# Sunscreen-tech/Sunscreen

Hardware: NVIDIA H100
Metric: ciphertext mul+relin/sec (higher is better)
Workload: dtype u64

## Files before the change

### sunscreen_b200/csrc/b200_bfv.cu

```cuda
#include "../../include/b200_bfv.h"
#include "bfv_body.cuh"
#include "host_ctx.h"
#include "ntt_body.cuh"
#include "ntt_fp_body.cuh"
#include <atomic>
#include <cstdio>
#include <cstdlib>
#include <cstring>
#ifdef B200_EMU_HEADER
#include B200_EMU_HEADER
#else
#include <cuda_runtime.h>
#include <map>
#include <string>
#include <vector>
struct B200TraceRec
{
    const char *name;
    cudaEvent_t e0, e1;
};
static int g_trace_on = -1;
static std::vector<B200TraceRec> g_trace;
static const char *g_trace_name = nullptr;
static inline bool trace_on()
// ... 128 lines not shown
    const int r = (int)(t % R);
    const long long item = t / R;
    const PrimeDev P = ld_prime(r < L.k ? &L.q[r] : &L.bsk[r - L.k]);
    const int Pn = square ? sa : sa + sb;
    const int Dn = square ? 3 : sa + sb - 1;
    const u64 *A = ext + ((item * Pn) * R + r) * n;
    u64 *Dp = D + ((item * Dn) * R + r) * n;
    if (!square && (sa > 4 || sb > 4))
    {
        tensor_coeff_general(P, A, R * n, sa, A + (long long)sa * R * n, R * n, sb, Dp, R * n, c);
        return;
    }
    if (L.fp)
    {
        const double *pd = r < L.k ? &L.dq[2 * r] : &L.dbsk[2 * (r - L.k)];
        const double p = __ldg(pd), pinv = __ldg(pd + 1);
        if (square)
            square_coeff_fp(p, pinv, A, R * n, Dp, R * n, c);
        else
            tensor_coeff_fp(p, pinv, A, R * n, sa, A + (long long)sa * R * n, R * n, sb, Dp, R * n, c);
        return;
    }
    if (square)
        square_coeff(P, A, R * n, Dp, R * n, c);
    else
        tensor_coeff(P, A, R * n, sa, A + (long long)sa * R * n, R * n, sb, Dp, R * n, c);
}

template <int K>
__global__ void scale_kernel(const ScaleIntC<K> L, const u64 *D, int Dn, u64 *dst0, int split, u64 *dst1, long long n,
                             long long total)
{
    const long long idx = GLOBAL_IDX();
    if (idx >= total)
        return;
    const int R = K + L.nBsk;
    const long long c = idx % n;
    const long long t = idx / n;
    const int m = (int)(t % Dn);
    const long long item = t / Dn;
    const u64 *src = D + ((item * Dn + m) * R) * n;
    u64 *dst = m < split ? dst0 + ((item * split + m) * K) * n : dst1 + ((item * (Dn - split) + (m - split)) * K) * n;
    scale_coeff<K>(L, src, dst, n, c);
}

template <int K>
__global__ void ksmac_kernel(const PrimeDev *primes, const NttPrimeFp *fprimes, int use_fp, int special_idx, int key_rows,
                             const u64 *ks1, const u64 *key, u64 *ks2, long long n, long long total)
{
    const long long idx = GLOBAL_IDX();
    if (idx >= total)
        return;
    const long long c = idx % n;
    const long long t = idx / n;
    const int I = (int)(t % (K + 1));
    const long long item = t / (K + 1);
    const int prime_idx = I < K ? I : special_idx;
    const int key_res = I < K ? I : key_rows - 1;
    const PrimeDev P = ld_prime(&primes[prime_idx]);
    const u64 *ops = ks1 + ((item * (K + 1) + I) * K) * n;
    const u64 *kp = key + (long long)key_res * n;
    u64 *o0 = ks2 + ((item * 2 + 0) * (K + 1) + I) * n;
    u64 *o1 = ks2 + ((item * 2 + 1) * (K + 1) + I) * n;
    if (use_fp)
    {
        const double p = __ldg(&fprimes[prime_idx].p), pinv = __ldg(&fprimes[prime_idx].pinv);
        ksmac_coeff_fp<K>(p, pinv, ops, n, kp, 2LL * key_rows * n, (long long)key_rows * n, o0, o1, c);
        return;
    }
    ksmac_coeff<K>(P, ops, n, kp, 2LL * key_rows * n, (long long)key_rows * n, o0, o1, c);
}

#ifdef B200_EMU_HEADER
struct b200_u64x2
{
    u64 x, y;
};
static inline b200_u64x2 ldg2(const u64 *p) { return b200_u64x2{ p[0], p[1] }; }
static inline void stg2(u64 *p, u64 a, u64 b)
{
    p[0] = a;
    p[1] = b;
}
#else
typedef ulonglong2 b200_u64x2;
__device__ __forceinline__ ulonglong2 ldg2(const u64 *p) { return __ldg(reinterpret_cast<const b200_u64x2 *>(p)); }
__device__ __forceinline__ void stg2(u64 *p, u64 a, u64 b) { *reinterpret_cast<ulonglong2 *>(p) = make_ulonglong2(a, b); }
#endif

template <int K>
__global__ void lift_kernel_v2(const LiftFpC<K> L, const u64 *a, int sa, const u64 *b, int sb, u64 *ext, long long n, long long total)
{
    const long long idx = GLOBAL_IDX();
    if (idx >= total)
        return;
    const int P = sa + sb;
    const long long hn = n >> 1;
    const long long c = (idx % hn) * 2;
    const long long t = idx / hn;
    const int p = (int)(t % P);
    const long long item = t / P;
    const int R = K + L.nBsk;
    const u64 *src = p < sa ? a + (item * sa + p) * K * n : b + (item * sb + (p - sa)) * K * n;
    u64 *dst = ext + ((item * P + p) * R + K) * n;
    u64 xs[2][K], zs[2][K + 2];
#pragma unroll
    for (int i = 0; i < K; i++)
    {
        const b200_u64x2 v = ldg2(src + i * n + c);
        xs[0][i] = v.x;
        xs[1][i] = v.y;
    }
    lift_coeff_fp<K>(L, xs[0], zs[0], 1, 0);
    lift_coeff_fp<K>(L, xs[1], zs[1], 1, 0);
#pragma unroll
    for (int j = 0; j < K + 2; j++)
        if (j < L.nBsk)
            stg2(dst + j * n + c, zs[0][j], zs[1][j]);
}

__global__ void tensor_kernel_v2(const LevelDev L, const u64 *ext, u64 *D, long long n, long long total, int square)
{
    const long long idx = GLOBAL_IDX();
    if (idx >= total)
        return;
    const int R = L.k + L.nBsk;
    const long long hn = n >> 1;
    const long long c = (idx % hn) * 2;
    const long long t = idx / hn;
    const int r = (int)(t % R);
    const long long item = t / R;
    const double *pd = r < L.k ? &L.dq[2 * r] : &L.dbsk[2 * (r - L.k)];
    const double p = __ldg(pd), pinv = __ldg(pd + 1);
    const int Pn = square ? 2 : 4;
    const u64 *A = ext + ((item * Pn) * R + r) * n + c;
    u64 *Dp = D + ((item * 3) * R + r) * n + c;
    const long long ps = (long long)R * n;
    const b200_u64x2 a0 = ldg2(A), a1 = ldg2(A + ps);
    u64 in[2][4], out[2][3];
    in[0][0] = a0.x; in[1][0] = a0.y; in[0][1] = a1.x; in[1][1] = a1.y;
    if (!square)
    {
        const b200_u64x2 b0 = ldg2(A + 2 * ps), b1 = ldg2(A + 3 * ps);
        in[0][2] = b0.x; in[1][2] = b0.y; in[0][3] = b1.x; in[1][3] = b1.y;
    }
#pragma unroll
    for (int u = 0; u < 2; u++)
    {
        if (square)
            square_coeff_fp(p, pinv, in[u], 1, out[u], 1, 0);
        else
            tensor_coeff_fp(p, pinv, in[u], 1, 2, in[u] + 2, 1, 2, out[u], 1, 0);
    }
#pragma unroll
    for (int m = 0; m < 3; m++)
        stg2(Dp + m * ps, out[0][m], out[1][m]);
}

template <int K>
__global__ void scale_kernel_v2(const ScaleFpC<K> L, const u64 *D, int Dn, u64 *dst0, int split, u64 *dst1, long long n, long long total)
{
    const long long idx = GLOBAL_IDX();
    if (idx >= total)
        return;
    const int R = K + L.nBsk;
    const long long hn = n >> 1;
    const long long c = (idx % hn) * 2;
    const long long t = idx / hn;
    const int m = (int)(t % Dn);
    const long long item = t / Dn;
    const u64 *src = D + ((item * Dn + m) * R) * n + c;
    u64 *dst = (m < split ? dst0 + ((item * split + m) * K) * n : dst1 + ((item * (Dn - split) + (m - split)) * K) * n) + c;
    u64 in[2][2 * K + 2], out[2][K];
#pragma unroll
    for (int i = 0; i < 2 * K + 2; i++)
        if (i < R)
        {
            const b200_u64x2 v = ldg2(src + i * n);
            in[0][i] = v.x;
            in[1][i] = v.y;
        }
    scale_coeff_fp<K>(L, in[0], out[0], 1, 0);
    scale_coeff_fp<K>(L, in[1], out[1], 1, 0);
#pragma unroll
    for (int i = 0; i < K; i++)
        stg2(dst + i * n, out[0][i], out[1][i]);
}

template <int K>
__global__ void ksmac_kernel_v2(const NttPrimeFp *fprimes, int special_idx, int key_rows, const u64 *ks1, const u64 *key, u64 *ks2,
                                long long n, long long total)
{
    const long long idx = GLOBAL_IDX();
    if (idx >= total)
        return;
    const long long hn = n >> 1;
    const long long c = (idx % hn) * 2;
    const long long t = idx / hn;
    const int I = (int)(t % (K + 1));
    const long long item = t / (K + 1);
    const int prime_idx = I < K ? I : special_idx;
    const int key_res = I < K ? I : key_rows - 1;
    const double p = __ldg(&fprimes[prime_idx].p), pinv = __ldg(&fprimes[prime_idx].pinv);
    const u64 *ops = ks1 + ((item * (K + 1) + I) * K) * n + c;
    const u64 *kp = key + (long long)key_res * n + c;
    double acc[2][2] = { { 0.0, 0.0 }, { 0.0, 0.0 } };
#pragma unroll
    for (int J = 0; J < K; J++)
    {
        const b200_u64x2 x = ldg2(ops + J * n);
        const b200_u64x2 k0 = ldg2(kp + J * 2LL * key_rows * n), k1 = ldg2(kp + J * 2LL * key_rows * n + (long long)key_rows * n);
        const double x0 = fp_from_u64(x.x), x1 = fp_from_u64(x.y);
        acc[0][0] = B200_DADD(acc[0][0], fp_mulmod2(x0, fp_from_u64(k0.x), p, pinv));
        acc[0][1] = B200_DADD(acc[0][1], fp_mulmod2(x0, fp_from_u64(k1.x), p, pinv));
        acc[1][0] = B200_DADD(acc[1][0], fp_mulmod2(x1, fp_from_u64(k0.y), p, pinv));
        acc[1][1] = B200_DADD(acc[1][1], fp_mulmod2(x1, fp_from_u64(k1.y), p, pinv));
    }
    u64 *o0 = ks2 + ((item * 2 + 0) * (K + 1) + I) * n + c;
    u64 *o1 = ks2 + ((item * 2 + 1) * (K + 1) + I) * n + c;
    stg2(o0, fp_to_canonical(acc[0][0], p, pinv), fp_to_canonical(acc[1][0], p, pinv));
    stg2(o1, fp_to_canonical(acc[0][1], p, pinv), fp_to_canonical(acc[1][1], p, pinv));
}

template <int K>
__global__ void ksmoddown_kernel(const PrimeDev *primes, int special_idx, const u64 *inv_qsp, const u64 *ks2,
                                 const u64 *base0, long long base0_stride, const u64 *base1, long long base1_stride,
                                 u64 *dst, long long dst_item_stride, long long n, long long total)
{
    const long long idx = GLOBAL_IDX();
    if (idx >= total)
        return;
    const long long c = idx % n;
    const long long t = idx / n;
    const int comp = (int)(t & 1);
    const long long item = t >> 1;
    const PrimeDev SP = ld_prime(&primes[special_idx]);
    const u64 *acc = ks2 + ((item * 2 + comp) * (K + 1)) * n;
    const u64 *base = comp == 0 ? (base0 ? base0 + item * base0_stride : nullptr)
                                : (base1 ? base1 + item * base1_stride : nullptr);
    u64 *d = dst + item * dst_item_stride + (long long)comp * K * n;
    ksmoddown_coeff<K>(primes, SP, inv_qsp, acc, n, base, d, c);
}

template <int K>
__global__ void ksmoddown_kernel_v2(const PrimeDev *primes, int special_idx, const u64 *inv_qsp, const u64 *ks2,
                                    const u64 *base0, long long base0_stride, const u64 *base1, long long base1_stride,
                                    u64 *dst, long long dst_item_stride, long long n, long long total)
{
    const long long idx = GLOBAL_IDX();
    if (idx >= total)
        return;
    const long long hn = n >> 1;
    const long long c = (idx % hn) * 2;
    const long long t = idx / hn;
    const int comp = (int)(t & 1);
    const long long item = t >> 1;
    const PrimeDev SP = ld_prime(&primes[special_idx]);
    const u64 *acc = ks2 + ((item * 2 + comp) * (K + 1)) * n + c;
    const u64 *base = comp == 0 ? (base0 ? base0 + item * base0_stride : nullptr) : (base1 ? base1 + item * base1_stride : nullptr);
    u64 *d = dst + item * dst_item_stride + (long long)comp * K * n + c;
    const u64 half = SP.p >> 1;
    const b200_u64x2 sp = ldg2(acc + (long long)K * n);
    u64 s0 = sp.x + half, s1 = sp.y + half;
    s0 = s0 >= SP.p ? s0 - SP.p : s0;
    s1 = s1 >= SP.p ? s1 - SP.p : s1;
#pragma unroll
    for (int i = 0; i < K; i++)
    {
        const PrimeDev Q = ld_prime(&primes[i]);
        const u64 h = barrett64(half, Q.p, Q.r1);
        const u64 w = B200_LDG(&inv_qsp[2 * i]), wq = B200_LDG(&inv_qsp[2 * i + 1]);
        const b200_u64x2 a = ldg2(acc + (long long)i * n);
        u64 v0 = a.x + (Q.p - barrett64(s0, Q.p, Q.r1)) + h;
        u64 v1 = a.y + (Q.p - barrett64(s1, Q.p, Q.r1)) + h;
        v0 = shoup_mul(v0, w, wq, Q.p);
        v1 = shoup_mul(v1, w, wq, Q.p);
        if (base)
        {
            const b200_u64x2 b = ldg2(base + c + (long long)i * n);
            v0 = add_mod(v0, b.x, Q.p);
            v1 = add_mod(v1, b.y, Q.p);
        }
        stg2(d + (long long)i * n, v0, v1);
    }
}

template <int K>
__global__ void modswitch_kernel(const PrimeDev *primes, const u64 *inv_qlast, const u64 *src, u64 *dst, long long n,
                                 long long total)
{
    const long long idx = GLOBAL_IDX();
    if (idx >= total)
        return;
    const long long c = idx % n;
    const long long poly = idx / n;
    modswitch_coeff<K>(primes, inv_qlast, src + poly * K * n, n, dst + poly * (K - 1) * n, c);
}

__global__ void galois_kernel(const PrimeDev *primes, int k, const u64 *in2, u64 *out2, u64 *tmp, int logn, u32 g,
                              long long total)
{
    const long long idx = GLOBAL_IDX();
    if (idx >= total)
        return;
    const long long n = 1LL << logn;
    const long long c = idx & (n - 1);
    const long long t = idx >> logn;
    const int r = (int)(t % k);
    const long long u = t / k;
    const int poly = (int)(u & 1);
    const long long item = u >> 1;
    const u64 p = __ldg(&primes[r].p);
    const u64 *src = in2 + ((item * 2 + poly) * k + r) * n;
    u64 *dst = poly == 0 ? out2 + ((item * 2) * k + r) * n : tmp + (item * k + r) * n;
    galois_coeff(p, src, dst, logn, g, c);
}

__global__ void addsub_kernel(const PrimeDev *primes, int k, const u64 *a, const u64 *b, u64 *out, int logn, int mode,
                              long long total)
{
    const long long idx = GLOBAL_IDX();
    if (idx >= total)
        return;
    const int r = (int)((idx >> logn) % k);
    const u64 p = __ldg(&primes[r].p);
    const u64 x = a[idx];
    u64 v;
    if (mode == 0)
        v = add_mod(x, b[idx], p);
    else if (mode == 1)
        v = sub_mod(x, b[idx], p);
    else
        v = neg_mod(x, p);
    out[idx] = v;
}

__global__ void expand_signed_kernel(const PrimeDev *primes, int k, const long long *vals, u64 *out, int logn, long long total)
{
    const long long idx = GLOBAL_IDX();
    if (idx >= total)
        return;
    const long long c = idx & ((1LL << logn) - 1);
    const long long row = idx >> logn;
    const int r = (int)(row % k);
    const long long poly = row / k;
    const long long v = vals[(poly << logn) + c];
    out[idx] = v < 0 ? __ldg(&primes[r].p) + (u64)v : (u64)v;
}

__global__ void dyadic_plain_kernel(const PrimeDev *primes, int k, int size, const u64 *x, const u64 *y, long long pb,
                                    u64 *out, int logn, long long total)
{
    const long long idx = GLOBAL_IDX();
    if (idx >= total)
        return;
    const long long n = 1LL << logn;
    const long long c = idx & (n - 1);
    const long long t = idx >> logn;
    const int r = (int)(t % k);
    const long long u = t / k;
    const long long item = u / size;
    const PrimeDev P = ld_prime(&primes[r]);
    const u64 yv = y[((item % pb) * k + r) * n + c];
    u64 lo, hi;
    mul128(x[idx], yv, lo, hi);
    out[idx] = barrett128(lo, hi, P.p, P.r0, P.r1);
}
// ... 919 lines not shown
    for (int b = 0; b < Lh.nB; b++)
    {
        C.sk_c[2 * b] = Lh.sk_c[b].w;
        C.sk_c[2 * b + 1] = Lh.sk_c[b].wq;
        C.sk_mat_msk[b] = Lh.sk_mat_msk[b];
    }
    C.sk_inv_b_msk = Lh.sk_inv_b_msk;
    return C;
}
template <int K>
static LiftFpC<K> make_lift_fpc(const b200_ctx *ctx, int level)
{
    const LevelFpHost &H = ctx->fp_levels[level];
    LiftFpC<K> C;
    memset(&C, 0, sizeof(C));
    C.nBsk = H.nBsk;
    C.neg_inv_q_mod_mt = H.neg_inv_q_mod_mt;
    for (int i = 0; i < K; i++)
        C.mt[i] = H.lift_mt[i];
    std::copy(H.dq.begin(), H.dq.end(), C.dq);
    std::copy(H.dbsk.begin(), H.dbsk.end(), C.dbsk);
    std::copy(H.lift_c.begin(), H.lift_c.end(), C.c);
    std::copy(H.lift_mat.begin(), H.lift_mat.end(), C.mat);
    std::copy(H.lift_qm.begin(), H.lift_qm.end(), C.qm);
    return C;
}
template <int K>
static ScaleFpC<K> make_scale_fpc(const b200_ctx *ctx, int level)
{
    const LevelFpHost &H = ctx->fp_levels[level];
    ScaleFpC<K> C;
    memset(&C, 0, sizeof(C));
    C.nB = H.nB;
    C.nBsk = H.nBsk;
    std::copy(H.dq.begin(), H.dq.end(), C.dq);
    std::copy(H.dbsk.begin(), H.dbsk.end(), C.dbsk);
    std::copy(H.scale_c.begin(), H.scale_c.end(), C.c);
    std::copy(H.scale_tq.begin(), H.scale_tq.end(), C.tq);
    std::copy(H.scale_mat.begin(), H.scale_mat.end(), C.mat);
    std::copy(H.sk_c.begin(), H.sk_c.end(), C.sk_c);
    for (int i = 0; i < K; i++)
        for (int b = 0; b < H.nB; b++)
        {
            C.sk_mat_q[2 * (i * (K + 1) + b)] = H.sk_mat_q[2 * (i * H.nB + b)];
            C.sk_mat_q[2 * (i * (K + 1) + b) + 1] = H.sk_mat_q[2 * (i * H.nB + b) + 1];
        }
    std::copy(H.sk_mat_msk.begin(), H.sk_mat_msk.end(), C.sk_mat_msk);
    std::copy(H.prod_b_q.begin(), H.prod_b_q.end(), C.prod_b_q);
    std::copy(H.negprod_b_q.begin(), H.negprod_b_q.end(), C.negprod_b_q);
    C.inv_b_msk[0] = H.inv_b_msk[0];
    C.inv_b_msk[1] = H.inv_b_msk[1];
    return C;
}

static const int EB = 256;

static int check_level(b200_ctx *ctx, int level)
{
    if (!ctx)
        return fail(B200_E_NULL, "null context");
    if (level < 0 || level >= (int)ctx->levels.size())
        return fail(B200_E_INVALID, "level out of range");
    return 0;
}

static int dense_job(b200_ctx *ctx, const std::string &key, const std::vector<int> &prime, JobDesc *jd)
{
    std::vector<long long> off(prime.size());
    for (size_t i = 0; i < prime.size(); i++)
        off[i] = (long long)i * (long long)ctx->n;
    return get_job(ctx, key, prime, off, off, jd);
}

static std::vector<int> row_primes(b200_ctx *ctx, int level, bool with_bsk)
{
    const LevelHost &Lh = ctx->host->levels[level];
    std::vector<int> r(Lh.q_idx);
    if (with_bsk)
        r.insert(r.end(), Lh.bsk_idx.begin(), Lh.bsk_idx.end());
    return r;
}

static int multiply_core(b200_ctx *ctx, int level, const u64 *a, int sa, const u64 *b, int sb, bool square, u64 *dst0,
                         int split, u64 *dst1, long long batch, cudaStream_t s)
{
    const LevelDev &L = ctx->levels[level];
    const LevelHost &Lh = ctx->host->levels[level];
    const long long n = (long long)ctx->n;
    const int k = L.k, R = k + L.nBsk;
    const int P = square ? sa : sa + sb;
    const int Dn = square ? 3 : sa + sb - 1;
    Scratch scr(ctx, s);
    u64 *ext = nullptr, *D = nullptr;
    int rc;
    if ((rc = scr.get((size_t)batch * P * R * n, &ext)))
        return rc;
    if ((rc = scr.get((size_t)batch * Dn * R * n, &D)))
        return rc;
    bool clustered = false;
    {
        if (L.fp)
        {
            const long long total = batch * P * (n >> 1);
            DISPATCH_K(k, B200_LAUNCH(lift_kernel_v2<KK>, blocks_for(total, EB), EB, 0, s, make_lift_fpc<KK>(ctx, level), a, sa,
                                      square ? a : b, square ? 0 : sb, ext, n, total));
        }
        else
        {
            const long long total = batch * P * n;
            DISPATCH_K(k, B200_LAUNCH(lift_kernel<KK>, blocks_for(total, EB), EB, 0, s, make_lift_intc<KK>(ctx, level), a, sa,
                                      square ? a : b, square ? 0 : sb, ext, n, total));
        }
        ctx->launches++;
    }
#ifndef B200_EMU_HEADER
    static const bool want_cluster = !(std::getenv("B200_MUL_CLUSTER") && std::getenv("B200_MUL_CLUSTER")[0] == '0') &&
                                     !std::getenv("B200_TENSOR_FUSION");
    if (want_cluster && !square && sa == 2 && sb == 2 && L.fp && ctx->mul_clusters > 0 && ctx->logn <= 13 &&
        4LL * R * batch > 2LL * ctx->sm_count)
    {
        JobDesc jd;
        if ((rc = get_job(ctx, "mulcl:" + std::to_string(level), row_primes(ctx, level, true), {}, {}, &jd)))
            return rc;
        if (static_fp_ok(ctx, jd))
        {
            if (4LL * R * batch > 0x7fffffffLL)
                return fail(B200_E_INVALID, "batch too large for one multiply launch");
            NttJob job;
            memset(&job, 0, sizeof(job));
            job.logn = ctx->logn;
            job.slots = R;
            job.slot_prime = jd.d_prime;
            job.primes = ctx->d_ntt_primes;
            job.fprimes = ctx->d_fp_primes;
            job.items = batch;
            cudaEvent_t t0 = nullptr, t1 = nullptr;
            if (trace_on())
            {
                cudaEventCreate(&t0);
                cudaEventCreate(&t1);
                cudaEventRecord(t0, s);
            }
            const int crc = b200_mul_cluster(ctx->logn, job, a, b, ext, D, k, s);
            if (crc)
                return fail(B200_E_CUDA, std::string("mul_cluster_kernel: ") + cudaGetErrorString((cudaError_t)crc));
            if (t0)
            {
                cudaEventRecord(t1, s);
                g_trace.push_back(B200TraceRec{ "mul_cluster_kernel", t0, t1 });
            }
            ctx->launches++;
            clustered = true;
        }
    }
#endif
    if (!clustered)
    {
        std::vector<int> prime;
        std::vector<long long> so, dof;
        NttAlt alt;
        for (int which = 0; which < (square ? 1 : 2); which++)
        {
            const int sz = which == 0 ? sa : sb;
            const int p0 = which == 0 ? 0 : sa;
            for (int p = 0; p < sz; p++)
                for (int r = 0; r < k; r++)
                {
                    prime.push_back(Lh.q_idx[r]);
                    so.push_back(((long long)p * k + r) * n);
                    dof.push_back(((long long)(p0 + p) * R + r) * n);
                }
            alt.end[which] = (int)prime.size();
            alt.src[which] = which == 0 ? a : b;
            alt.stride[which] = (long long)sz * k * n;
        }
        if (square)
            alt.end[1] = alt.end[0];
        for (int p = 0; p < P; p++)
            for (int j = 0; j < L.nBsk; j++)
            {
                prime.push_back(Lh.bsk_idx[j]);
                so.push_back(((long long)p * R + k + j) * n);
                dof.push_back(((long long)p * R + k + j) * n);
            }
        JobDesc jd;
        std::string key = "mulfwd:" + std::to_string(level) + ":" + std::to_string(sa) + ":" + std::to_string(square ? 0 : sb);
        if ((rc = get_job(ctx, key, prime, so, dof, &jd)))
            return rc;
        if ((rc = launch_ntt<true>(ctx, jd, ext, (long long)P * R * n, ext, (long long)P * R * n, batch, 0, s, nullptr, &alt)))
            return rc;
    }
    if (!clustered)
    {
        std::vector<int> rows = row_primes(ctx, level, true), prime;
        for (int m = 0; m < Dn; m++)
            prime.insert(prime.end(), rows.begin(), rows.end());
        JobDesc jd;
        if ((rc = dense_job(ctx, "muld:" + std::to_string(level) + ":" + std::to_string(Dn), prime, &jd)))
            return rc;
        static const bool want_fuse = std::getenv("B200_TENSOR_FUSION") != nullptr;
        const bool fuse = want_fuse && L.fp && static_fp_ok(ctx, jd);
        TensorArgs ta;
        if (fuse)
        {
            ta.mode = square ? 2 : 1;
            ta.sa = sa;
            ta.sb = sb;
            ta.rows = R;
            ta.src = ext;
        }
        else
        {
            if (L.fp && (square || (sa == 2 && sb == 2)))
            {
                const long long total = batch * R * (n >> 1);
                B200_LAUNCH(tensor_kernel_v2, blocks_for(total, EB), EB, 0, s, L, ext, D, n, total, square ? 1 : 0);
            }
            else
            {
                const long long total = batch * R * n;
                B200_LAUNCH(tensor_kernel, blocks_for(total, EB), EB, 0, s, L, ext, sa, sb, D, n, total, square ? 1 : 0);
            }
            ctx->launches++;
        }
        if ((rc = launch_ntt<false>(ctx, jd, D, (long long)Dn * R * n, D, (long long)Dn * R * n, batch, 0, s, fuse ? &ta : nullptr)))
            return rc;
    }
    {
        if (L.fp)
        {
            const long long total = batch * Dn * (n >> 1);
            DISPATCH_K(k, B200_LAUNCH(scale_kernel_v2<KK>, blocks_for(total, EB), EB, 0, s, make_scale_fpc<KK>(ctx, level), D, Dn,
                                      dst0, split, dst1, n, total));
        }
        else
        {
            const long long total = batch * Dn * n;
            DISPATCH_K(k, B200_LAUNCH(scale_kernel<KK>, blocks_for(total, EB), EB, 0, s, make_scale_intc<KK>(ctx, level), D, Dn, dst0,
                                      split, dst1, n, total));
        }
        ctx->launches++;
    }
    CU_TRY(cudaGetLastError());
    return 0;
}

static int keyswitch_core(b200_ctx *ctx, int level, const u64 *d, long long d_stride, const u64 *key, const u64 *base0,
                          long long base0_stride, const u64 *base1, long long base1_stride, u64 *dst,
                          long long dst_stride, long long batch, cudaStream_t s)
{
    if (!ctx->host->using_keyswitching || level < 1)
        return fail(B200_E_LOGIC, "keyswitching is not supported by the context");
    const LevelDev &L = ctx->levels[level];
    const LevelHost &Lh = ctx->host->levels[level];
    const long long n = (long long)ctx->n;
    const int k = L.k;
    const int Kkey = ctx->host->K;
    const int special = Kkey - 1;
    Scratch scr(ctx, s);
    u64 *ks1 = nullptr, *ks2 = nullptr;
    int rc;
    if ((rc = scr.get((size_t)batch * 2 * (k + 1) * n, &ks2)))
        return rc;
    bool clustered = false;
#ifndef B200_EMU_HEADER
    static const bool want_cluster = !(std::getenv("B200_KS_CLUSTER") && std::getenv("B200_KS_CLUSTER")[0] == '0');
    if (want_cluster && L.fp && ctx->logn <= 13 && k >= 2 && k <= 8 && ctx->ks_clusters[k] > 0 &&
        (long long)k * (k + 1) * batch > 2LL * ctx->sm_count)
    {
        std::vector<int> prime;
        for (int I = 0; I <= k; I++)
            prime.push_back(I < k ? Lh.q_idx[I] : special);
        JobDesc jd;
        if ((rc = get_job(ctx, "kscl:" + std::to_string(level), prime, {}, {}, &jd)))
            return rc;
        if (static_fp_ok(ctx, jd))
        {
            if ((long long)k * (k + 1) * batch > 0x7fffffffLL)
                return fail(B200_E_INVALID, "batch too large for one key-switch launch");
            NttJob job;
            memset(&job, 0, sizeof(job));
            job.logn = ctx->logn;
            job.slots = k + 1;
            job.slot_prime = jd.d_prime;
            job.primes = ctx->d_ntt_primes;
            job.fprimes = ctx->d_fp_primes;
            job.reduce_input = 1;
            job.items = batch;
            cudaEvent_t t0 = nullptr, t1 = nullptr;
            if (trace_on())
            {
                cudaEventCreate(&t0);
                cudaEventCreate(&t1);
                cudaEventRecord(t0, s);
            }
            const int crc = b200_ks_cluster(ctx->logn, job, d, d_stride, key, Kkey, ks2, k, s);
            if (crc)
                return fail(B200_E_CUDA, std::string("ks_cluster_kernel: ") + cudaGetErrorString((cudaError_t)crc));
            if (t0)
            {
                cudaEventRecord(t1, s);
                g_trace.push_back(B200TraceRec{ "ks_cluster_kernel", t0, t1 });
            }
            ctx->launches++;
            clustered = true;
        }
    }
#endif
    if (!clustered && (rc = scr.get((size_t)batch * (k + 1) * k * n, &ks1)))
        return rc;
    if (!clustered)
    {
        std::vector<int> prime;
        std::vector<long long> so, dof;
        for (int I = 0; I <= k; I++)
            for (int J = 0; J < k; J++)
            {
                prime.push_back(I < k ? Lh.q_idx[I] : special);
                so.push_back((long long)J * n);
                dof.push_back(((long long)I * k + J) * n);
            }
        JobDesc jd;
        if ((rc = get_job(ctx, "ks1:" + std::to_string(level), prime, so, dof, &jd)))
            return rc;
        if ((rc = launch_ntt<true>(ctx, jd, d, d_stride, ks1, (long long)(k + 1) * k * n, batch, 1, s)))
            return rc;
    }
    if (!clustered)
    {
        bool done = false;
#ifndef B200_EMU_HEADER
        static const bool want_tma = !(std::getenv("B200_KSMAC_TMA") && std::getenv("B200_KSMAC_TMA")[0] == '0');
        if (want_tma && b200_ksmac_tma_supported(n, k))
        {
            if (trace_on())
                g_trace_name = "ksmac_tma_kernel";
            cudaEvent_t t0 = nullptr, t1 = nullptr;
            if (trace_on())
            {
                cudaEventCreate(&t0);
                cudaEventCreate(&t1);
                cudaEventRecord(t0, s);
            }
            const int rc2 = b200_ksmac_tma(k, L.fp ? 1 : 0, ctx->d_primes, ctx->d_fp_primes, special, Kkey, ks1, key, ks2, n, batch,
                                           ctx->sm_count, s);
            if (rc2 > 0)
                return fail(B200_E_CUDA, std::string("ksmac_tma_kernel: ") + cudaGetErrorString((cudaError_t)rc2));
            if (rc2 == 0)
            {
                done = true;
                if (t0)
                {
                    cudaEventRecord(t1, s);
                    g_trace.push_back(B200TraceRec{ "ksmac_tma_kernel", t0, t1 });
                    g_trace_name = nullptr;
                }
            }
        }
#endif
        if (done)
            ;
        else if (L.fp)
        {
            const long long total = batch * (k + 1) * (n >> 1);
            DISPATCH_K(k, B200_LAUNCH(ksmac_kernel_v2<KK>, blocks_for(total, EB), EB, 0, s, ctx->d_fp_primes, special, Kkey, ks1, key,
                                      ks2, n, total));
        }
        else
        {
            const long long total = batch * (k + 1) * n;
            DISPATCH_K(k, B200_LAUNCH(ksmac_kernel<KK>, blocks_for(total, EB), EB, 0, s, ctx->d_primes, ctx->d_fp_primes,
                                      (int)(L.fp != 0), special, Kkey, ks1, key, ks2, n, total));
        }
        ctx->launches++;
    }
    if (!clustered)
    {
        std::vector<int> prime;
        for (int comp = 0; comp < 2; comp++)
            for (int I = 0; I <= k; I++)
                prime.push_back(I < k ? Lh.q_idx[I] : special);
        JobDesc jd;
        if ((rc = dense_job(ctx, "ks2:" + std::to_string(level), prime, &jd)))
            return rc;
        if ((rc = launch_ntt<false>(ctx, jd, ks2, 2LL * (k + 1) * n, ks2, 2LL * (k + 1) * n, batch, 0, s)))
            return rc;
    }
    {
        const long long total = batch * 2 * (n >> 1);
        DISPATCH_K(k, B200_LAUNCH(ksmoddown_kernel_v2<KK>, blocks_for(total, EB), EB, 0, s, ctx->d_primes, special, ctx->d_inv_qsp, ks2,
                                                                                base0, base0_stride, base1, base1_stride,
                                                                                dst, dst_stride, n, total));
        ctx->launches++;
    }
    CU_TRY(cudaGetLastError());
    return 0;
}

extern "C" {

const char *b200_last_error(void) { return g_err.c_str(); }

int b200_device_count(void)
{
    int c = 0;
    if (cudaGetDeviceCount(&c) != cudaSuccess)
        return 0;
    return c;
}

int b200_ctx_create(uint64_t n, const uint64_t *coeff_modulus, uint64_t count, uint64_t plain_modulus, int device,
                    b200_ctx **out)
{
    if (!coeff_modulus || !out)
        return fail(B200_E_NULL, "null argument");
    *out = nullptr;
    std::unique_ptr<b200_ctx> ctx(new b200_ctx());
    try
    {
        std::vector<b200::u64> mods(coeff_modulus, coeff_modulus + count);
        ctx->host.reset(new BfvHostContext((size_t)n, mods, plain_modulus));
    }
    catch (const std::invalid_argument &e)
    {
        return fail(B200_E_INVALID, e.what());
    }
    catch (const std::logic_error &e)
    {
        return fail(B200_E_LOGIC, e.what());
    }
    catch (const std::exception &e)
    {
        return fail(B200_E_INVALID, e.what());
    }
    ctx->n = ctx->host->n;
    ctx->logn = ctx->host->logn;
    int ndev = 0;
    cudaError_t e = cudaGetDeviceCount(&ndev);
    if (e != cudaSuccess || ndev == 0)
        return fail(B200_E_CUDA, "no CUDA device available: the CUDA backend has no CPU fallback");
    if (device < 0 || device >= ndev)
        return fail(B200_E_INVALID, "device index out of range");
    CU_TRY(cudaSetDevice(device));
    ctx->device = device;
    cudaDeviceProp prop;
    CU_TRY(cudaGetDeviceProperties(&prop, device));
    ctx->sm_count = prop.multiProcessorCount;
    ctx->ntt_split = ctx->logn >= 15 ? (std::getenv("B200_NTT_SPLIT") ? atoi(std::getenv("B200_NTT_SPLIT")) : 2) : 0;
    if (ctx->ntt_split < 1 && ctx->logn >= 15)
        ctx->ntt_split = 1;
    if (ctx->ntt_split > 2)
        ctx->ntt_split = 2;
    if (ctx->logn > 15)
        return fail(B200_E_INVALID, "poly_modulus_degree above 32768 is not supported");
    const int local_logn = ctx->logn - ctx->ntt_split;
    ctx->npass = ntt_schedule(local_logn, ctx->pass_L);
    ctx->ntt_smem = (size_t)ntt_smem_words(1 << local_logn) * sizeof(u64);
    if (ctx->ntt_smem > (size_t)prop.sharedMemPerBlockOptin)
        return fail(B200_E_INVALID, "poly_modulus_degree too large for the shared-memory NTT");
    ctx->ntt_threads = local_logn >= 14 ? 512 : (local_logn >= 10 ? 256 : 64);
#ifndef B200_EMU_HEADER
    {
        const int frc = b200_ntt_fp_setup((int)prop.sharedMemPerBlockOptin);
        if (frc)
            return fail(B200_E_CUDA, std::string("cudaFuncSetAttribute (FP64 NTT kernels): ") + cudaGetErrorString((cudaError_t)frc));
        const int crc = b200_mul_cluster_setup(ctx->logn, &ctx->mul_clusters);
        if (crc)
            return fail(B200_E_CUDA, std::string("mul_cluster_kernel setup: ") + cudaGetErrorString((cudaError_t)crc));
        for (int k = 2; k <= 8; k++)
        {
            const int krc = b200_ks_cluster_setup(ctx->logn, k, &ctx->ks_clusters[k]);
            if (krc)
                return fail(B200_E_CUDA, std::string("ks_cluster_kernel setup: ") + cudaGetErrorString((cudaError_t)krc));
        }
    }
// ... 550 lines not shown
int b200_expand_signed(b200_ctx *ctx, int level, const int64_t *vals, int polys, uint64_t *out, void *stream)
{
    int rc = check_level(ctx, level);
    if (rc)
        return rc;
    if (!vals || !out)
        return fail(B200_E_NULL, "null pointer");
    if (polys < 1)
        return 0;
    CU_TRY(cudaSetDevice(ctx->device));
    const int k = ctx->levels[level].k;
    const long long total = (long long)polys * k * (long long)ctx->n;
    B200_LAUNCH(expand_signed_kernel, blocks_for(total, EB), EB, 0, (cudaStream_t)stream, ctx->d_primes, k, (const long long *)vals,
                (u64 *)out, ctx->logn, total);
    ctx->launches++;
    CU_TRY(cudaGetLastError());
    return 0;
}

int b200_multiply(b200_ctx *ctx, int level, const uint64_t *a, int sa, const uint64_t *b, int sb, uint64_t *out,
                  uint64_t batch, void *stream)
{
    int rc = check_level(ctx, level);
    if (rc)
        return rc;
    if (!a || !b || !out)
        return fail(B200_E_NULL, "null ciphertext pointer");
    if (sa < 1 || sb < 1 || sa + sb - 1 > 16)
        return fail(B200_E_INVALID, "ciphertext sizes must be >= 1 with a destination size of at most 16");
    if (batch == 0)
        return 0;
    CU_TRY(cudaSetDevice(ctx->device));
    const int Dn = sa + sb - 1;
    return multiply_core(ctx, level, (const u64 *)a, sa, (const u64 *)b, sb, false, (u64 *)out, Dn, nullptr,
                         (long long)batch, (cudaStream_t)stream);
}

int b200_square(b200_ctx *ctx, int level, const uint64_t *a, uint64_t *out, uint64_t batch, void *stream)
{
    int rc = check_level(ctx, level);
    if (rc)
        return rc;
    if (!a || !out)
        return fail(B200_E_NULL, "null ciphertext pointer");
    if (batch == 0)
        return 0;
    CU_TRY(cudaSetDevice(ctx->device));
    return multiply_core(ctx, level, (const u64 *)a, 2, nullptr, 0, true, (u64 *)out, 3, nullptr, (long long)batch,
                         (cudaStream_t)stream);
}

int b200_relinearize(b200_ctx *ctx, int level, const uint64_t *in3, const uint64_t *relin_key, uint64_t *out2,
                     uint64_t batch, void *stream)
{
    int rc = check_level(ctx, level);
    if (rc)
        return rc;
    if (!in3 || !relin_key || !out2)
        return fail(B200_E_NULL, "null pointer");
    if (batch == 0)
        return 0;
    if ((const void *)in3 == (const void *)out2 && batch != 1)
        return fail(B200_E_INVALID, "in-place relinearize is only defined for batch == 1");
    CU_TRY(cudaSetDevice(ctx->device));
    const long long n = (long long)ctx->n;
    const int k = ctx->levels[level].k;
    const u64 *c = (const u64 *)in3;
    return keyswitch_core(ctx, level, c + 2LL * k * n, 3LL * k * n, (const u64 *)relin_key, c, 3LL * k * n, c + (long long)k * n,
                          3LL * k * n, (u64 *)out2, 2LL * k * n, (long long)batch, (cudaStream_t)stream);
}

static int multiply_relin_one(b200_ctx *ctx, int level, const uint64_t *a, const uint64_t *b, const uint64_t *relin_key,
                             uint64_t *out2, uint64_t batch, void *stream)
{
    int rc = check_level(ctx, level);
    if (rc)
        return rc;
    if (!a || !b || !relin_key || !out2)
        return fail(B200_E_NULL, "null pointer");
    if (batch == 0)
        return 0;
    CU_TRY(cudaSetDevice(ctx->device));
    const long long n = (long long)ctx->n;
    const int k = ctx->levels[level].k;
    cudaStream_t s = (cudaStream_t)stream;
    Scratch scr(ctx, s);
    u64 *c2 = nullptr;
    if ((rc = scr.get((size_t)batch * k * n, &c2)))
        return rc;
    if ((rc = multiply_core(ctx, level, (const u64 *)a, 2, (const u64 *)b, 2, false, (u64 *)out2, 2, c2, (long long)batch, s)))
        return rc;
    u64 *o = (u64 *)out2;
    return keyswitch_core(ctx, level, c2, (long long)k * n, (const u64 *)relin_key, o, 2LL * k * n, o + (long long)k * n,
                          2LL * k * n, o, 2LL * k * n, (long long)batch, s);
}

int b200_multiply_relin(b200_ctx *ctx, int level, const uint64_t *a, const uint64_t *b, const uint64_t *relin_key,
                        uint64_t *out2, uint64_t batch, void *stream)
{
    int rc = check_level(ctx, level);
    if (rc)
        return rc;
    const int parts = (ctx->mr_split > 1 && batch >= 64) ? ctx->mr_split : 1;
    if (parts == 1)
        return multiply_relin_one(ctx, level, a, b, relin_key, out2, batch, stream);
    CU_TRY(cudaSetDevice(ctx->device));
    cudaStream_t us = (cudaStream_t)stream;
    const size_t w = (size_t)2 * ctx->levels[level].k * ctx->n;
    CU_TRY(cudaEventRecord(ctx->ev_fork, us));
    for (int p = 0; p < parts && !rc; p++)
    {
        const uint64_t lo = batch * p / parts, hi = batch * (p + 1) / parts;
        CU_TRY(cudaStreamWaitEvent(ctx->s_side[p], ctx->ev_fork, 0));
        rc = multiply_relin_one(ctx, level, a + lo * w, b + lo * w, relin_key, out2 + lo * w, hi - lo, ctx->s_side[p]);
        CU_TRY(cudaEventRecord(ctx->ev_join[p], ctx->s_side[p]));
        CU_TRY(cudaStreamWaitEvent(us, ctx->ev_join[p], 0));
    }
    return rc;
}

int b200_apply_galois(b200_ctx *ctx, int level, const uint64_t *in2, uint32_t galois_elt, const uint64_t *galois_key,
                      uint64_t *out2, uint64_t batch, void *stream)
{
    int rc = check_level(ctx, level);
    if (rc)
        return rc;
    if (!in2 || !galois_key || !out2)
        return fail(B200_E_NULL, "null pointer");
    if (!(galois_elt & 1) || galois_elt >= 2 * ctx->n)
        return fail(B200_E_INVALID, "Galois element is not valid");
    if ((const void *)in2 == (const void *)out2)
        return fail(B200_E_INVALID, "apply_galois cannot run in place at this layer");
    if (batch == 0)
        return 0;
    CU_TRY(cudaSetDevice(ctx->device));
    const long long n = (long long)ctx->n;
    const LevelDev &L = ctx->levels[level];
    const int k = L.k;
    cudaStream_t s = (cudaStream_t)stream;
    Scratch scr(ctx, s);
    u64 *tmp = nullptr;
    if ((rc = scr.get((size_t)batch * k * n, &tmp)))
        return rc;
    const long long total = (long long)batch * 2 * k * n;
    B200_LAUNCH(galois_kernel, blocks_for(total, EB), EB, 0, s, ctx->d_primes, k, (const u64 *)in2, (u64 *)out2, tmp, ctx->logn,
                                                       galois_elt, total);
    ctx->launches++;
    u64 *o = (u64 *)out2;
    return keyswitch_core(ctx, level, tmp, (long long)k * n, (const u64 *)galois_key, o, 2LL * k * n, nullptr, 0, o,
                          2LL * k * n, (long long)batch, s);
}

int b200_multiply_plain(b200_ctx *ctx, int level, const uint64_t *a, int size, const uint64_t *plain, uint64_t pb,
                        uint64_t *out, uint64_t batch, void *stream)
{
    int rc = check_level(ctx, level);
    if (rc)
        return rc;
    if (!a || !plain || !out)
        return fail(B200_E_NULL, "null pointer");
    if (size < 1 || (pb != 1 && pb != batch))
        return fail(B200_E_INVALID, "size / plain_batch");
    if (batch == 0)
        return 0;
    CU_TRY(cudaSetDevice(ctx->device));
    const long long n = (long long)ctx->n;
    const LevelDev &L = ctx->levels[level];
    const int k = L.k;
    cudaStream_t s = (cudaStream_t)stream;
    Scratch scr(ctx, s);
    u64 *pl = nullptr;
    if ((rc = scr.get((size_t)pb * k * n, &pl)))
        return rc;
    u32 *mono = nullptr;
    if (L.fast_plain_lift)
// ... 819 lines not shown
```

Before: 90880.

## Fuse BFV scale-down of c0/c1 into keyswitch moddown kernel for mul+relin

In multiply+relinearize, the tensor product buffer D is kept alive and only the c2 component is scaled in multiply_core. The c0/c1 scaling is deferred and fused into a new scale_moddown kernel that computes the scaled base in registers and adds it during the keyswitch mod-down. This avoids writing the scaled c0/c1 to the output and reading them back, at the cost of holding the extended-basis D in scratch longer and higher register pressure. It is gated by a heuristic on k versus R.

```diff
diff --git a/sunscreen_b200/csrc/b200_bfv.cu b/sunscreen_b200/csrc/b200_bfv.cu
--- a/sunscreen_b200/csrc/b200_bfv.cu
+++ b/sunscreen_b200/csrc/b200_bfv.cu
@@ -234,10 +234,12 @@
     p[0] = a;
     p[1] = b;
 }
+#define B200_DEV static inline
 #else
 typedef ulonglong2 b200_u64x2;
 __device__ __forceinline__ ulonglong2 ldg2(const u64 *p) { return __ldg(reinterpret_cast<const b200_u64x2 *>(p)); }
 __device__ __forceinline__ void stg2(u64 *p, u64 a, u64 b) { *reinterpret_cast<ulonglong2 *>(p) = make_ulonglong2(a, b); }
+#define B200_DEV __device__ __forceinline__
 #endif
 
 template <int K>
@@ -310,7 +312,25 @@
 }
 
 template <int K>
-__global__ void scale_kernel_v2(const ScaleFpC<K> L, const u64 *D, int Dn, u64 *dst0, int split, u64 *dst1, long long n, long long total)
+B200_DEV void scale2_fp(const ScaleFpC<K> &L, const u64 *src, long long n, u64 (&out)[2][K])
+{
+    const int R = K + L.nBsk;
+    u64 in[2][2 * K + 2];
+#pragma unroll
+    for (int i = 0; i < 2 * K + 2; i++)
+        if (i < R)
+        {
+            const b200_u64x2 v = ldg2(src + i * n);
+            in[0][i] = v.x;
+            in[1][i] = v.y;
+        }
+    scale_coeff_fp<K>(L, in[0], out[0], 1, 0);
+    scale_coeff_fp<K>(L, in[1], out[1], 1, 0);
+}
+
+template <int K>
+__global__ void scale_kernel_v2(const ScaleFpC<K> L, const u64 *D, int Dn, int m0, u64 *dst0, int split, u64 *dst1, long long n,
+                                long long total)
 {
     const long long idx = GLOBAL_IDX();
     if (idx >= total)
@@ -319,21 +339,11 @@
     const long long hn = n >> 1;
     const long long c = (idx % hn) * 2;
     const long long t = idx / hn;
-    const int m = (int)(t % Dn);
-    const long long item = t / Dn;
-    const u64 *src = D + ((item * Dn + m) * R) * n + c;
+    const int m = m0 + (int)(t % (Dn - m0));
+    const long long item = t / (Dn - m0);
     u64 *dst = (m < split ? dst0 + ((item * split + m) * K) * n : dst1 + ((item * (Dn - split) + (m - split)) * K) * n) + c;
-    u64 in[2][2 * K + 2], out[2][K];
-#pragma unroll
-    for (int i = 0; i < 2 * K + 2; i++)
-        if (i < R)
-        {
-            const b200_u64x2 v = ldg2(src + i * n);
-            in[0][i] = v.x;
-            in[1][i] = v.y;
-        }
-    scale_coeff_fp<K>(L, in[0], out[0], 1, 0);
-    scale_coeff_fp<K>(L, in[1], out[1], 1, 0);
+    u64 out[2][K];
+    scale2_fp<K>(L, D + ((item * Dn + m) * R) * n + c, n, out);
 #pragma unroll
     for (int i = 0; i < K; i++)
         stg2(dst + i * n, out[0][i], out[1][i]);
@@ -395,6 +405,31 @@
 }
 
 template <int K>
+B200_DEV void ksmoddown2(const PrimeDev *primes, int special_idx, const u64 *inv_qsp, const u64 *acc, long long n,
+                         const u64 (&base)[2][K], u64 *d)
+{
+    const PrimeDev SP = ld_prime(&primes[special_idx]);
+    const u64 half = SP.p >> 1;
+    const b200_u64x2 sp = ldg2(acc + (long long)K * n);
+    u64 s0 = sp.x + half, s1 = sp.y + half;
+    s0 = s0 >= SP.p ? s0 - SP.p : s0;
+    s1 = s1 >= SP.p ? s1 - SP.p : s1;
+#pragma unroll
+    for (int i = 0; i < K; i++)
+    {
+        const PrimeDev Q = ld_prime(&primes[i]);
+        const u64 h = barrett64(half, Q.p, Q.r1);
+        const u64 w = B200_LDG(&inv_qsp[2 * i]), wq = B200_LDG(&inv_qsp[2 * i + 1]);
+        const b200_u64x2 a = ldg2(acc + (long long)i * n);
+        u64 v0 = a.x + (Q.p - barrett64(s0, Q.p, Q.r1)) + h;
+        u64 v1 = a.y + (Q.p - barrett64(s1, Q.p, Q.r1)) + h;
+        v0 = shoup_mul(v0, w, wq, Q.p);
+        v1 = shoup_mul(v1, w, wq, Q.p);
+        stg2(d + (long long)i * n, add_mod(v0, base[0][i], Q.p), add_mod(v1, base[1][i], Q.p));
+    }
+}
+
+template <int K>
 __global__ void ksmoddown_kernel_v2(const PrimeDev *primes, int special_idx, const u64 *inv_qsp, const u64 *ks2,
                                     const u64 *base0, long long base0_stride, const u64 *base1, long long base1_stride,
                                     u64 *dst, long long dst_item_stride, long long n, long long total)
@@ -407,34 +442,35 @@
     const long long t = idx / hn;
     const int comp = (int)(t & 1);
     const long long item = t >> 1;
-    const PrimeDev SP = ld_prime(&primes[special_idx]);
-    const u64 *acc = ks2 + ((item * 2 + comp) * (K + 1)) * n + c;
     const u64 *base = comp == 0 ? (base0 ? base0 + item * base0_stride : nullptr) : (base1 ? base1 + item * base1_stride : nullptr);
-    u64 *d = dst + item * dst_item_stride + (long long)comp * K * n + c;
-    const u64 half = SP.p >> 1;
-    const b200_u64x2 sp = ldg2(acc + (long long)K * n);
-    u64 s0 = sp.x + half, s1 = sp.y + half;
-    s0 = s0 >= SP.p ? s0 - SP.p : s0;
-    s1 = s1 >= SP.p ? s1 - SP.p : s1;
+    u64 b[2][K];
 #pragma unroll
     for (int i = 0; i < K; i++)
     {
-        const PrimeDev Q = ld_prime(&primes[i]);
-        const u64 h = barrett64(half, Q.p, Q.r1);
-        const u64 w = B200_LDG(&inv_qsp[2 * i]), wq = B200_LDG(&inv_qsp[2 * i + 1]);
-        const b200_u64x2 a = ldg2(acc + (long long)i * n);
-        u64 v0 = a.x + (Q.p - barrett64(s0, Q.p, Q.r1)) + h;
-        u64 v1 = a.y + (Q.p - barrett64(s1, Q.p, Q.r1)) + h;
-        v0 = shoup_mul(v0, w, wq, Q.p);
-        v1 = shoup_mul(v1, w, wq, Q.p);
-        if (base)
-        {
-            const b200_u64x2 b = ldg2(base + c + (long long)i * n);
-            v0 = add_mod(v0, b.x, Q.p);
-            v1 = add_mod(v1, b.y, Q.p);
-        }
-        stg2(d + (long long)i * n, v0, v1);
-    }
+        const b200_u64x2 v = base ? ldg2(base + c + (long long)i * n) : b200_u64x2{ 0, 0 };
+        b[0][i] = v.x;
+        b[1][i] = v.y;
+    }
+    ksmoddown2<K>(primes, special_idx, inv_qsp, ks2 + ((item * 2 + comp) * (K + 1)) * n + c, n, b,
+                  dst + item * dst_item_stride + (long long)comp * K * n + c);
+}
+
+template <int K>
+__global__ void scale_moddown_kernel_v2(const ScaleFpC<K> L, const PrimeDev *primes, int special_idx, const u64 *inv_qsp,
+                                        const u64 *D, const u64 *ks2, u64 *dst, long long n, long long total)
+{
+    const long long idx = GLOBAL_IDX();
+    if (idx >= total)
+        return;
+    const long long hn = n >> 1;
+    const long long c = (idx % hn) * 2;
+    const long long t = idx / hn;
+    const int comp = (int)(t & 1);
+    const long long item = t >> 1;
+    u64 b[2][K];
+    scale2_fp<K>(L, D + ((item * 3 + comp) * (K + L.nBsk)) * n + c, n, b);
+    ksmoddown2<K>(primes, special_idx, inv_qsp, ks2 + ((item * 2 + comp) * (K + 1)) * n + c, n, b,
+                  dst + (item * 2 + comp) * K * n + c);
 }
 
 template <int K>
@@ -1520,7 +1556,7 @@
 }
 
 static int multiply_core(b200_ctx *ctx, int level, const u64 *a, int sa, const u64 *b, int sb, bool square, u64 *dst0,
-                         int split, u64 *dst1, long long batch, cudaStream_t s)
+                         int split, u64 *dst1, long long batch, cudaStream_t s, u64 *keep_D = nullptr)
 {
     const LevelDev &L = ctx->levels[level];
     const LevelHost &Lh = ctx->host->levels[level];
@@ -1529,11 +1565,11 @@
     const int P = square ? sa : sa + sb;
     const int Dn = square ? 3 : sa + sb - 1;
     Scratch scr(ctx, s);
-    u64 *ext = nullptr, *D = nullptr;
+    u64 *ext = nullptr, *D = keep_D;
     int rc;
     if ((rc = scr.get((size_t)batch * P * R * n, &ext)))
         return rc;
-    if ((rc = scr.get((size_t)batch * Dn * R * n, &D)))
+    if (!D && (rc = scr.get((size_t)batch * Dn * R * n, &D)))
         return rc;
     bool clustered = false;
     {
@@ -1667,9 +1703,10 @@
     {
         if (L.fp)
         {
-            const long long total = batch * Dn * (n >> 1);
+            const int m0 = keep_D ? split : 0;
+            const long long total = batch * (Dn - m0) * (n >> 1);
             DISPATCH_K(k, B200_LAUNCH(scale_kernel_v2<KK>, blocks_for(total, EB), EB, 0, s, make_scale_fpc<KK>(ctx, level), D, Dn,
-                                      dst0, split, dst1, n, total));
+                                      m0, dst0, split, dst1, n, total));
         }
         else
         {
@@ -1685,7 +1722,7 @@
 
 static int keyswitch_core(b200_ctx *ctx, int level, const u64 *d, long long d_stride, const u64 *key, const u64 *base0,
                           long long base0_stride, const u64 *base1, long long base1_stride, u64 *dst,
-                          long long dst_stride, long long batch, cudaStream_t s)
+                          long long dst_stride, long long batch, cudaStream_t s, const u64 *D = nullptr)
 {
     if (!ctx->host->using_keyswitching || level < 1)
         return fail(B200_E_LOGIC, "keyswitching is not supported by the context");
@@ -1826,9 +1863,17 @@
     }
     {
         const long long total = batch * 2 * (n >> 1);
-        DISPATCH_K(k, B200_LAUNCH(ksmoddown_kernel_v2<KK>, blocks_for(total, EB), EB, 0, s, ctx->d_primes, special, ctx->d_inv_qsp, ks2,
-                                                                                base0, base0_stride, base1, base1_stride,
-                                                                                dst, dst_stride, n, total));
+        if (D)
+        {
+            DISPATCH_K(k, B200_LAUNCH(scale_moddown_kernel_v2<KK>, blocks_for(total, EB), EB, 0, s, make_scale_fpc<KK>(ctx, level),
+                                      ctx->d_primes, special, ctx->d_inv_qsp, D, ks2, dst, n, total));
+        }
+        else
+        {
+            DISPATCH_K(k, B200_LAUNCH(ksmoddown_kernel_v2<KK>, blocks_for(total, EB), EB, 0, s, ctx->d_primes, special, ctx->d_inv_qsp, ks2,
+                                                                                    base0, base0_stride, base1, base1_stride,
+                                                                                    dst, dst_stride, n, total));
+        }
         ctx->launches++;
     }
     CU_TRY(cudaGetLastError());
@@ -2545,15 +2590,25 @@
         return 0;
     CU_TRY(cudaSetDevice(ctx->device));
     const long long n = (long long)ctx->n;
-    const int k = ctx->levels[level].k;
+    const LevelDev &L = ctx->levels[level];
+    const int k = L.k, R = k + L.nBsk;
     cudaStream_t s = (cudaStream_t)stream;
     Scratch scr(ctx, s);
-    u64 *c2 = nullptr;
+    u64 *c2 = nullptr, *D = nullptr;
     if ((rc = scr.get((size_t)batch * k * n, &c2)))
         return rc;
-    if ((rc = multiply_core(ctx, level, (const u64 *)a, 2, (const u64 *)b, 2, false, (u64 *)out2, 2, c2, (long long)batch, s)))
-        return rc;
     u64 *o = (u64 *)out2;
+    if (L.fp && (k + 1) * (k + 2) <= 4 * R)
+    {
+        if ((rc = scr.get((size_t)batch * 3 * R * n, &D)))
+            return rc;
+        if ((rc = multiply_core(ctx, level, (const u64 *)a, 2, (const u64 *)b, 2, false, nullptr, 2, c2, (long long)batch, s, D)))
+            return rc;
+        return keyswitch_core(ctx, level, c2, (long long)k * n, (const u64 *)relin_key, nullptr, 0, nullptr, 0, o, 2LL * k * n,
+                              (long long)batch, s, D);
+    }
+    if ((rc = multiply_core(ctx, level, (const u64 *)a, 2, (const u64 *)b, 2, false, o, 2, c2, (long long)batch, s)))
+        return rc;
     return keyswitch_core(ctx, level, c2, (long long)k * n, (const u64 *)relin_key, o, 2LL * k * n, o + (long long)k * n,
                           2LL * k * n, o, 2LL * k * n, (long long)batch, s);
 }
```

After: 94180, median of 6. 1.04x the previous value.
